# rueberger/MJHMC

Measured on AMD Instinct MI355X. Metric: particle-steps/sec (ndims x nparticles x L), higher is better.
Workload: dtype f64 state (ProductOfT: around the f32 matrix-core force)

## Files before the change

mjhmc_amd/csrc/dense_pot64_kernels.hpp:

```cpp
#pragma once
#ifndef __HIPCC_RTC__
#include <hip/hip_runtime.h>
#endif
#include <stdint.h>

#include "dense_pot.hpp"
#include "dense_pot_tile.hpp"

namespace mjhmc {

template <int NB>
struct DVecN;
template <>
struct DVecN<1> {
  using type = double;
};
template <>
struct DVecN<2> {
  using type = __attribute__((ext_vector_type(2))) double;
};
template <>
struct DVecN<4> {
  using type = __attribute__((ext_vector_type(4))) double;
};
// ... 11 lines not shown
template <int NB>
__device__ __forceinline__ int q_off(int q) { return NB * ((q & 3) + 8 * (q >> 2)); }
template <int NB>
__device__ __forceinline__ const double* lane_row(const double* base, int64_t p, int w, int h) {
  return base + (size_t)p * (128 * NB) + 32 * NB * w + 4 * NB * h;
}
template <int NB>
__device__ __forceinline__ double* lane_row(double* base, int64_t p, int w, int h) {
  return base + (size_t)p * (128 * NB) + 32 * NB * w + 4 * NB * h;
}
template <int NB>
__device__ __forceinline__ typename DVecN<NB>::type dv_load(const double* lrow, int q) {
  return *reinterpret_cast<const typename DVecN<NB>::type*>(lrow + q_off<NB>(q));
}
template <int NB>
__device__ __forceinline__ void dv_store(double* lrow, int q, const typename DVecN<NB>::type& v) {
  *reinterpret_cast<typename DVecN<NB>::type*>(lrow + q_off<NB>(q)) = v;
}

constexpr int kPark = 8;
template <int NB>
struct Shared64 {
  Shared<NB> s;
  double red64[4][kP];
  double zn[128 * NB];
  f32x4 park[kPark / 2][256];
};

template <int NB>
struct Work {
  static constexpr int PB = NB == 1 ? 8 : 16;
  static constexpr int PQ = NB * 8 / PB;
  static constexpr unsigned kArea = 16u * PQ * 64u * PB;
  __amdgpu_buffer_rsrc_t rs;
  unsigned voff;
  static constexpr unsigned xb = 0;
  static constexpr unsigned vb = 4 * kArea;
};
template <int NB>
__device__ __forceinline__ Work<NB> work_of(double* scratch, unsigned wg, int w, int lane) {
  Work<NB> k;
  char* base = (char*)scratch + (size_t)wg * (8 * Work<NB>::kArea);
  k.rs = __builtin_amdgcn_make_buffer_rsrc((void*)base, 0, 8 * Work<NB>::kArea, 0x00020000);
  k.voff = (unsigned)w * Work<NB>::kArea + (unsigned)lane * Work<NB>::PB;
  return k;
}
using uvec4 = __attribute__((ext_vector_type(4))) unsigned;
using uvec2 = __attribute__((ext_vector_type(2))) unsigned;
using f64x2 = __attribute__((ext_vector_type(2))) double;
template <int NB>
__device__ __forceinline__ typename DVecN<NB>::type wk_load(const Work<NB>& k, unsigned area, int q) {
  if constexpr (NB == 1) {
    return __builtin_bit_cast(double, __builtin_amdgcn_raw_buffer_load_b64(k.rs, k.voff, area + (unsigned)q * 512u, 0));
  } else if constexpr (NB == 2) {
    return __builtin_bit_cast(f64x2, __builtin_amdgcn_raw_buffer_load_b128(k.rs, k.voff, area + (unsigned)q * 1024u, 0));
  } else {
    const f64x2 lo = __builtin_bit_cast(f64x2, __builtin_amdgcn_raw_buffer_load_b128(k.rs, k.voff, area + (unsigned)q * 2048u, 0));
    const f64x2 hi = __builtin_bit_cast(f64x2, __builtin_amdgcn_raw_buffer_load_b128(k.rs, k.voff, area + (unsigned)q * 2048u + 1024u, 0));
    typename DVecN<4>::type v;
    v[0] = lo[0];
    v[1] = lo[1];
    v[2] = hi[0];
    v[3] = hi[1];
    return v;
  }
}
template <int NB>
__device__ __forceinline__ void wk_store(const Work<NB>& k, unsigned area, int q, const typename DVecN<NB>::type& v) {
  if constexpr (NB == 1) {
    __builtin_amdgcn_raw_buffer_store_b64(__builtin_bit_cast(uvec2, v), k.rs, k.voff, area + (unsigned)q * 512u, 0);
  } else if constexpr (NB == 2) {
    __builtin_amdgcn_raw_buffer_store_b128(__builtin_bit_cast(uvec4, v), k.rs, k.voff, area + (unsigned)q * 1024u, 0);
  } else {
    f64x2 lo, hi;
    lo[0] = v[0];
    lo[1] = v[1];
    hi[0] = v[2];
    hi[1] = v[3];
    __builtin_amdgcn_raw_buffer_store_b128(__builtin_bit_cast(uvec4, lo), k.rs, k.voff, area + (unsigned)q * 2048u, 0);
    __builtin_amdgcn_raw_buffer_store_b128(__builtin_bit_cast(uvec4, hi), k.rs, k.voff, area + (unsigned)q * 2048u + 1024u, 0);
  }
}

template <int NB>
struct PieceOf {
  using type = uvec4;
};
template <>
struct PieceOf<1> {
  using type = unsigned long long;
};
template <int NB>
struct Stage {
  using P = typename PieceOf<NB>::type;
  static constexpr int PB = sizeof(P);
  static constexpr int RB = 1024 * NB;
  static constexpr int RP = RB / PB;
  static constexpr int K = 32 * RP / 256;
  static constexpr int KB = K < 16 ? K : 16;
};
__device__ __forceinline__ unsigned stage_addr(int row, int piece, int pb, int rb) {
  return (unsigned)(row * rb + ((piece ^ (row & 15)) * pb));
}
template <int NB>
__device__ __forceinline__ void stage_rows_in(const double* rows, int64_t p, char* img) {
  using S = Stage<NB>;
  using P = typename S::P;
  const int t = threadIdx.x;
#pragma unroll 1
  for (int i0 = 0; i0 < S::K; i0 += S::KB) {
    P buf[S::KB];
#pragma unroll
    for (int i = 0; i < S::KB; ++i) {
      const int k = (i0 + i) * 256 + t, row = k / S::RP, piece = k % S::RP;
      const int64_t pr = __shfl((long long)p, row);
      buf[i] = *reinterpret_cast<const P*>(reinterpret_cast<const char*>(rows) + (size_t)pr * S::RB + (size_t)piece * S::PB);
    }
#pragma unroll
    for (int i = 0; i < S::KB; ++i) {
      const int k = (i0 + i) * 256 + t, row = k / S::RP, piece = k % S::RP;
      *reinterpret_cast<P*>(img + stage_addr(row, piece, S::PB, S::RB)) = buf[i];
    }
  }
}
template <int NB>
__device__ __forceinline__ void stage_rows_out(double* rows, int64_t p, const char* img) {
  using S = Stage<NB>;
  using P = typename S::P;
  const int t = threadIdx.x;
#pragma unroll 1
  for (int i0 = 0; i0 < S::K; i0 += S::KB) {
#pragma unroll
    for (int i = 0; i < S::KB; ++i) {
      const int k = (i0 + i) * 256 + t, row = k / S::RP, piece = k % S::RP;
      const int64_t pr = __shfl((long long)p, row);
      *reinterpret_cast<P*>(reinterpret_cast<char*>(rows) + (size_t)pr * S::RB + (size_t)piece * S::PB) =
          *reinterpret_cast<const P*>(img + stage_addr(row, piece, S::PB, S::RB));
    }
  }
}
template <int NB>
__device__ __forceinline__ typename DVecN<NB>::type stage_get(const char* img, int w, int c, int h, int q) {
  using S = Stage<NB>;
  const int first = (8 * NB * (32 * w + acc_row(q, h))) / S::PB;
  if constexpr (NB == 4) {
    const f64x2 lo = *reinterpret_cast<const f64x2*>(img + stage_addr(c, first, S::PB, S::RB));
    const f64x2 hi = *reinterpret_cast<const f64x2*>(img + stage_addr(c, first + 1, S::PB, S::RB));
    typename DVecN<4>::type v;
    v[0] = lo[0];
    v[1] = lo[1];
    v[2] = hi[0];
    v[3] = hi[1];
    return v;
  } else {
    return *reinterpret_cast<const typename DVecN<NB>::type*>(img + stage_addr(c, first, S::PB, S::RB));
  }
}
template <int NB>
__device__ __forceinline__ void stage_put(char* img, int w, int c, int h, int q, const typename DVecN<NB>::type& v) {
  using S = Stage<NB>;
  const int first = (8 * NB * (32 * w + acc_row(q, h))) / S::PB;
  if constexpr (NB == 4) {
    f64x2 lo, hi;
    lo[0] = v[0];
    lo[1] = v[1];
    hi[0] = v[2];
    hi[1] = v[3];
    *reinterpret_cast<f64x2*>(img + stage_addr(c, first, S::PB, S::RB)) = lo;
    *reinterpret_cast<f64x2*>(img + stage_addr(c, first + 1, S::PB, S::RB)) = hi;
  } else {
    *reinterpret_cast<typename DVecN<NB>::type*>(img + stage_addr(c, first, S::PB, S::RB)) = v;
  }
}
template <int NB>
__device__ __forceinline__ char* stage_image(Shared<NB>& s) {
  static_assert(sizeof(s.pub) == 32 * Stage<NB>::RB, "the staging image is the two B-operand images");
  return reinterpret_cast<char*>(&s.pub[0][0]);
}

template <int NB>
struct VTile {
  double b[NB][16];
};

template <int NB, int NKICK>
__device__ __forceinline__ void kick_drift_pass(const Work<NB>& wk, const Tile<NB>& g, VTile<NB>& v, double c, double eps,
                                                PubWave<NB>* pub0, int w, int lane) {
  using DV = typename DVecN<NB>::type;
  DV xa[4], xb[4];
  auto load4 = [&](int q4, DV(&x)[4]) {
#pragma unroll
    for (int qq = 0; qq < 4; ++qq) x[qq] = wk_load<NB>(wk, wk.xb, 4 * q4 + qq);
  };
  auto kick4 = [&](int q4) {
#pragma unroll
    for (int qq = 0; qq < 4; ++qq) {
      const int q = 4 * q4 + qq;
#pragma unroll
      for (int r = 0; r < NB; ++r) {
        const double t = c * (double)g.b[r][q];
        double vv = v.b[r][q];
        vv = vv + t;
        if constexpr (NKICK == 2) vv = vv + t;
        v.b[r][q] = vv;
      }
    }
  };
  auto drift4 = [&](int q4, DV(&x)[4]) {
    f32x4 px[NB];
#pragma unroll
    for (int qq = 0; qq < 4; ++qq) {
      const int q = 4 * q4 + qq;
#pragma unroll
      for (int r = 0; r < NB; ++r) {
        const double xx = dget<NB>(x[qq], r) + eps * v.b[r][q];
        dset<NB>(x[qq], r, xx);
        px[r][qq] = (float)xx;
      }
      wk_store<NB>(wk, wk.xb, q, x[qq]);
    }
    if constexpr (NB == 4) {
      unsigned off = ((wk.voff >> 1) & 0xFFFFC000u) | (wk.voff & 0x3FFu);
      asm volatile("" : "+v"(off));
      char* img = reinterpret_cast<char*>(pub0) + off;
#pragma unroll
      for (int r = 0; r < NB; ++r) *reinterpret_cast<f32x4*>(img + (size_t)(r * 4 + q4) * 1024) = px[r];
    } else {
#pragma unroll
      for (int r = 0; r < NB; ++r) pub0[w].v[r][q4][lane] = px[r];
    }
  };
  load4(0, xa);
  load4(1, xb);
  __builtin_amdgcn_sched_barrier(0);
  kick4(0);
  drift4(0, xa);
  __builtin_amdgcn_sched_barrier(0);
  load4(2, xa);
  __builtin_amdgcn_sched_barrier(0);
  kick4(1);
  drift4(1, xb);
  __builtin_amdgcn_sched_barrier(0);
  load4(3, xb);
  __builtin_amdgcn_sched_barrier(0);
  kick4(2);
  drift4(2, xa);
  __builtin_amdgcn_sched_barrier(0);
  kick4(3);
  drift4(3, xb);
}

template <int NB>
__device__ __forceinline__ double closing_kick(const Tile<NB>& g, VTile<NB>& v, double c) {
  double s = 0.0;
#pragma unroll
  for (int q = 0; q < 16; ++q)
#pragma unroll
    for (int r = 0; r < NB; ++r) {
      const double vv = v.b[r][q] + c * (double)g.b[r][q];
      v.b[r][q] = vv;
      s = s + vv * vv;
    }
  return s;
}

template <int NB, class SH>
__device__ __forceinline__ double column_sum(SH& sh, int w, int c, int h, double part) {
  const double both = swap32_sum(part);
  if (h == 0) sh.red64[w][c] = both;
  __syncthreads();
  const double tot = sh.red64[0][c] + sh.red64[1][c] + sh.red64[2][c] + sh.red64[3][c];
  __syncthreads();
  return tot;
}

template <int NB>
__device__ __forceinline__ void staged_start(Shared<NB>& s, const Work<NB>& wk, const double* xin, const double* vin,
                                             const double* gin, int64_t p, int w, int c, int h, Tile<NB>& g, VTile<NB>& v,
                                             bool neg) {
  char* img = stage_image<NB>(s);
  stage_rows_in<NB>(xin, p, img);
  __syncthreads();
#pragma unroll
  for (int q = 0; q < 16; ++q) wk_store<NB>(wk, wk.xb, q, stage_get<NB>(img, w, c, h, q));
  __syncthreads();
  stage_rows_in<NB>(gin, p, img);
  __syncthreads();
#pragma unroll
  for (int q = 0; q < 16; ++q) {
    const typename DVecN<NB>::type gg = stage_get<NB>(img, w, c, h, q);
#pragma unroll
    for (int r = 0; r < NB; ++r) g.b[r][q] = (float)dget<NB>(gg, r);
  }
  __syncthreads();
  stage_rows_in<NB>(vin, p, img);
  __syncthreads();
#pragma unroll
  for (int q = 0; q < 16; ++q) {
    const typename DVecN<NB>::type vv = stage_get<NB>(img, w, c, h, q);
#pragma unroll
    for (int r = 0; r < NB; ++r) v.b[r][q] = neg ? -dget<NB>(vv, r) : dget<NB>(vv, r);
  }
  __syncthreads();
}

template <int NB>
__device__ __forceinline__ void staged_end_x(Shared<NB>& s, const Work<NB>& wk, double* xout, int64_t p, int w, int c, int h) {
  char* img = stage_image<NB>(s);
#pragma unroll
  for (int q = 0; q < 16; ++q) stage_put<NB>(img, w, c, h, q, wk_load<NB>(wk, wk.xb, q));
  __syncthreads();
  stage_rows_out<NB>(xout, p, img);
  __syncthreads();
}
template <int NB>
__device__ __forceinline__ void staged_end_vg(Shared<NB>& s, double* vout, double* gout, int64_t p, int w, int c, int h,
                                              const VTile<NB>& v, const Tile<NB>& g) {
  using DV = typename DVecN<NB>::type;
  char* img = stage_image<NB>(s);
#pragma unroll
  for (int q = 0; q < 16; ++q) {
    DV vv;
#pragma unroll
    for (int r = 0; r < NB; ++r) dset<NB>(vv, r, v.b[r][q]);
    stage_put<NB>(img, w, c, h, q, vv);
  }
  __syncthreads();
  stage_rows_out<NB>(vout, p, img);
  __syncthreads();
#pragma unroll
  for (int q = 0; q < 16; ++q) {
    DV gg;
#pragma unroll
    for (int r = 0; r < NB; ++r) dset<NB>(gg, r, (double)g.b[r][q]);
    stage_put<NB>(img, w, c, h, q, gg);
  }
  __syncthreads();
  stage_rows_out<NB>(gout, p, img);
  __syncthreads();
}

template <int NB, class XP>
__device__ __forceinline__ double pot64_trajectory(const PotModel& mdl, const XP& xp, AReg<NB>& ar, Shared64<NB>& sh, int w, int c, int h,
                                                   int lane, const Work<NB>& wk, Tile<NB>& g, VTile<NB>& v, int L, double eps,
                                                   double chalf, float* ex) {
  PubWave<NB>* pub0 = sh.s.pub[0];
  kick_drift_pass<NB, 1>(wk, g, v, chalf, eps, pub0, w, lane);
  for (int s = 0; s < L; ++s) {
    [[maybe_unused]] const int stamp_slot = s;
    POT_STAMP(0);
    if constexpr (NB == 4) {
#pragma unroll
      for (int k = 0; k < kPark / 2; ++k) {
        f64x2 two;
        two[0] = v.b[NB - 1][15 - 2 * k];
        two[1] = v.b[NB - 1][14 - 2 * k];
        sh.park[k][threadIdx.x] = __builtin_bit_cast(f32x4, two);
      }
    }
    pot_gradient_published<NB>(mdl, xp, ar, sh.s, w, c, h, lane, g, s == L - 1, ex, s);
    if constexpr (NB == 4) {
#pragma unroll
      for (int k = 0; k < kPark / 2; ++k) {
        const f64x2 two = __builtin_bit_cast(f64x2, sh.park[k][threadIdx.x]);
        v.b[NB - 1][15 - 2 * k] = two[0];
        v.b[NB - 1][14 - 2 * k] = two[1];
      }
#pragma unroll
      for (int r = 0; r < NB; ++r)
#pragma unroll
        for (int q = 0; q < 16; ++q) use_here(v.b[r][q]);
    }
    POT_STAMP(6);
    if (s < L - 1) kick_drift_pass<NB, 2>(wk, g, v, chalf, eps, pub0, w, lane);
    POT_STAMP(7);
  }
  const double part = closing_kick<NB>(g, v, chalf);
  return column_sum<NB>(sh, w, c, h, part) / 2.0;
}


template <int NB>
struct Finish64Shared {
  struct {
    int move[kP];
  } s;
  double red64[4][kP];
  double zn[128 * NB];
};

template <int NB, bool REPLAY, int MODE, bool FIX, class SH>
__device__ __forceinline__ void pot64_finish(const Pot64JumpArgs& a, SH& sh, int64_t p, bool alive, size_t roff, int w, int c,
                                             int h, const VTile<NB>& v, const Tile<NB>& g) {
  using DV = typename DVecN<NB>::type;
  const double* xin = a.X_in + roff;
  const double* vin = a.V_in + roff;
  const double* gin = a.G_in + roff;
  double* xo = a.X_out + roff;
  double* vo = a.V_out + roff;
  double* go = a.G_out + roff;
  const int mv = sh.s.move[c];
  const int k = mv & 3;
  bool take, flip, refresh;
  if constexpr (MODE == kModeControl) {
    const bool accept = k & 1, fl = k & 2;
    take = accept;
    flip = accept != fl;
    refresh = (mv & 4) != 0;
  } else {
    take = k == 0;
    flip = (MODE == kModeCT && k == 0) || k == 1;
    refresh = k == 2;
  }
  const bool tile_refreshes = __ballot(refresh) != 0ull;
  if (!FIX || !take) {
#pragma unroll
    for (int q = 0; q < 16; ++q) {
      DV gg;
      if (take) {
        if constexpr (!FIX) {
          DV vv;
#pragma unroll
          for (int r = 0; r < NB; ++r) {
            dset<NB>(vv, r, flip ? -v.b[r][q] : v.b[r][q]);
            dset<NB>(gg, r, (double)g.b[r][q]);
          }
          dv_store<NB>(vo, q, vv);
        }
      } else {
        gg = dv_load<NB>(gin, q);
        dv_store<NB>(xo, q, dv_load<NB>(xin, q));
      }
      dv_store<NB>(go, q, gg);
    }
  }
  double s2 = 0.0;
  if (!take || (REPLAY && refresh)) {
    const double* vsrc = take ? (const double*)vo : vin;
    const bool fl2 = flip && !take;
    const double* nrow = REPLAY ? lane_row<NB>(a.noise, alive ? p : 0, w, h) : nullptr;
#pragma unroll 1
    for (int q = 0; q < 16; ++q) {
      DV vv = dv_load<NB>(vsrc, q);
      if (fl2) vv = -vv;
      if constexpr (REPLAY) {
        if (refresh) {
          const DV z = dv_load<NB>(nrow, q);
#pragma unroll
          for (int r = 0; r < NB; ++r) {
            const double t = dget<NB>(vv, r) * a.r_keep + dget<NB>(z, r) * a.r_mix;
            dset<NB>(vv, r, t);
            s2 = s2 + t * t;
          }
        }
      }
      dv_store<NB>(vo, q, vv);
    }
// ... 80 lines not shown
```

mjhmc_amd/csrc/dense_pot_tile.hpp:

```cpp
#pragma once
#ifndef __HIPCC_RTC__
#include <hip/hip_runtime.h>
#endif
#include <stdint.h>

#include "dense_pot.hpp"
#include "timing_variants.hpp"

namespace mjhmc {

using f32x16 = __attribute__((ext_vector_type(16))) float;
using f32x4 = __attribute__((ext_vector_type(4))) float;

constexpr int kP = 32;

__device__ __forceinline__ int acc_row(int q, int h) { return (q & 3) + 8 * (q >> 2) + 4 * h; }

template <int NB>
struct Tile {
  f32x16 b[NB];
};

template <int NB>
struct VecN;
// ... 36 lines not shown
template <int NB>
__device__ __forceinline__ void tile_store(float* base, int64_t p, int w, int h, const Tile<NB>& t) {
  using V = typename VecN<NB>::type;
  float* row = base + (size_t)p * (128 * NB) + 32 * NB * w;
#pragma unroll
  for (int q = 0; q < 16; ++q) {
    V v;
#pragma unroll
    for (int r = 0; r < NB; ++r) vset<NB>(v, r, t.b[r][q]);
    *reinterpret_cast<V*>(row + NB * acc_row(q, h)) = v;
  }
}

template <int NB>
struct PubWave {
  f32x4 v[NB][4][64];
};

template <int NB>
__device__ __forceinline__ void publish(PubWave<NB>& dst, int lane, const Tile<NB>& t) {
#pragma unroll
  for (int r = 0; r < NB; ++r)
#pragma unroll
    for (int q4 = 0; q4 < 4; ++q4) {
      f32x4 v;
      v[0] = t.b[r][4 * q4 + 0];
      v[1] = t.b[r][4 * q4 + 1];
      v[2] = t.b[r][4 * q4 + 2];
      v[3] = t.b[r][4 * q4 + 3];
      dst.v[r][q4][lane] = v;
    }
}

template <int NB>
__device__ __forceinline__ void a_chunk_load(const float* mlane, int chunk, typename VecN<NB>::type (&dst)[16]) {
  using V = typename VecN<NB>::type;
  constexpr int DIM = 128 * NB;
  const float* base = mlane + (size_t)(32 * NB * (chunk / NB) + (chunk % NB)) * DIM;
#pragma unroll
  for (int q = 0; q < 16; ++q) dst[q] = *reinterpret_cast<const V*>(base + (size_t)(NB * ((q & 3) + 8 * (q >> 2))) * DIM);
}

template <int NB>
__device__ __forceinline__ typename VecN<NB>::type buf_load(__amdgpu_buffer_rsrc_t r, unsigned voff, unsigned soff) {
  using V = typename VecN<NB>::type;
  if constexpr (NB == 4) return __builtin_bit_cast(V, __builtin_amdgcn_raw_buffer_load_b128(r, voff, soff, 0));
  else if constexpr (NB == 2) return __builtin_bit_cast(V, __builtin_amdgcn_raw_buffer_load_b64(r, voff, soff, 0));
  else return __builtin_bit_cast(V, __builtin_amdgcn_raw_buffer_load_b32(r, voff, soff, 0));
}
template <int NB>
__device__ __forceinline__ __amdgpu_buffer_rsrc_t a_rsrc(const float* M) {
  constexpr int DIM = 128 * NB;
  return __builtin_amdgcn_make_buffer_rsrc((void*)M, 0, DIM * DIM * 4, 0x00020000);
}
template <int NB>
__device__ __forceinline__ void a_chunk_load_buf(__amdgpu_buffer_rsrc_t r, unsigned lane_bytes, int chunk,
                                                 typename VecN<NB>::type (&dst)[16]) {
  constexpr int DIM = 128 * NB;
  const unsigned cbase = (unsigned)(32 * NB * (chunk / NB) + (chunk % NB)) * (unsigned)(DIM * 4);
#pragma unroll
  for (int q = 0; q < 16; ++q) dst[q] = buf_load<NB>(r, lane_bytes, cbase + (unsigned)(NB * ((q & 3) + 8 * (q >> 2)) * DIM * 4));
}

template <int NB>
__device__ __forceinline__ void chunk_mfma(const f32x4* bbase, int chunk, int lane, const typename VecN<NB>::type (&a)[16],
                                           f32x4& bnext, Tile<NB>& acc) {
  constexpr int NG = 16 * NB;
#pragma unroll
  for (int q4 = 0; q4 < 4; ++q4) {
    const f32x4 b4 = bnext;
    const int t = 4 * chunk + q4 + 1;
    bnext = bbase[(size_t)(t < NG ? t : NG - 1) * 64 + lane];
    __builtin_amdgcn_sched_barrier(0);
#pragma unroll
    for (int qq = 0; qq < 4; ++qq) {
#pragma unroll
      for (int r = 0; r < NB; ++r)
        acc.b[r] = __builtin_amdgcn_mfma_f32_32x32x2f32(vget<NB>(a[4 * q4 + qq], r), b4[qq], acc.b[r], 0, 0, 0);
    }
    __builtin_amdgcn_sched_barrier(0);
  }
}

template <int NB>
__device__ __forceinline__ void chunk_mfma_ld(const f32x4* bbase, int chunk, int lane, const typename VecN<NB>::type (&a)[16],
                                              f32x4& bnext, Tile<NB>& acc, __amdgpu_buffer_rsrc_t rs, unsigned lane_bytes,
                                              unsigned cbase, typename VecN<NB>::type (&aload)[16]) {
  constexpr int NG = 16 * NB, DIM = 128 * NB;
#pragma unroll
  for (int q4 = 0; q4 < 4; ++q4) {
    const f32x4 b4 = bnext;
    const int t = 4 * chunk + q4 + 1;
    bnext = bbase[(size_t)(t < NG ? t : NG - 1) * 64 + lane];
    __builtin_amdgcn_sched_barrier(0);
#pragma unroll
    for (int qq = 0; qq < 4; ++qq) {
      const int q = 4 * q4 + qq;
#pragma unroll
      for (int r = 0; r < NB; ++r)
        acc.b[r] = __builtin_amdgcn_mfma_f32_32x32x2f32(vget<NB>(a[q], r), b4[qq], acc.b[r], 0, 0, 0);
      aload[q] = buf_load<NB>(rs, lane_bytes, cbase + (unsigned)(NB * ((q & 3) + 8 * (q >> 2)) * DIM * 4));
      __builtin_amdgcn_sched_barrier(0);
    }
    __builtin_amdgcn_sched_barrier(0);
  }
}

template <int NB>
__device__ __forceinline__ void gemm_dim(const float* __restrict__ M, const float* __restrict__ Mnext, const PubWave<NB>* pub,
                                         int w, int c, int h, int lane, typename VecN<NB>::type (&a0)[16], Tile<NB>& acc) {
  constexpr int DIM = 128 * NB, NCH = 4 * NB;
  const size_t lane_off = (size_t)(4 * NB * h) * DIM + 32 * NB * w + NB * c;
  const unsigned lane_bytes = (unsigned)(lane_off * sizeof(float));
  const __amdgpu_buffer_rsrc_t rM = a_rsrc<NB>(M), rN = a_rsrc<NB>(Mnext);
  const f32x4* bbase = &pub[0].v[0][0][0];
  typename VecN<NB>::type a1[16];
  f32x4 bnext = bbase[lane];
#pragma unroll 1
  for (int chunk = 0; chunk < NCH; chunk += 2) {
    const bool more = chunk + 2 < NCH;
    const int c1 = chunk + 1, c2 = more ? chunk + 2 : 0;
    chunk_mfma_ld<NB>(bbase, chunk, lane, a0, bnext, acc, rM, lane_bytes,
                      (unsigned)(32 * NB * (c1 / NB) + (c1 % NB)) * (unsigned)(DIM * 4), a1);
    chunk_mfma_ld<NB>(bbase, chunk + 1, lane, a1, bnext, acc, more ? rM : rN, lane_bytes,
                      (unsigned)(32 * NB * (c2 / NB) + (c2 % NB)) * (unsigned)(DIM * 4), a0);
  }
}

template <int NB>
struct AReg {
  typename VecN<NB>::type a0[16];
};
template <>
struct AReg<1> {
  float w1[4][16];
  float w2[4][16];
};

template <int NB>
__device__ __forceinline__ void areg_load(const PotModel& mdl, int w, int c, int h, AReg<NB>& ar) {
  if constexpr (NB == 1) {
    const float* m1 = mdl.W1 + (size_t)(4 * h) * 128 + 32 * w + c;
    const float* m2 = mdl.W2T + (size_t)(4 * h) * 128 + 32 * w + c;
#pragma unroll
    for (int chunk = 0; chunk < 4; ++chunk) {
      a_chunk_load<1>(m1, chunk, ar.w1[chunk]);
      a_chunk_load<1>(m2, chunk, ar.w2[chunk]);
    }
  } else {
    a_chunk_load<NB>(mdl.W1 + (size_t)(4 * NB * h) * (128 * NB) + 32 * NB * w + NB * c, 0, ar.a0);
  }
}

template <int NB, bool SECOND>
__device__ __forceinline__ void gemm_any(const PotModel& mdl, AReg<NB>& ar, const PubWave<NB>* pub, int w, int c,
                                         int h, int lane, Tile<NB>& acc) {
  if constexpr (NB == 1) {
    const int kdim = mdl.ndims;
#pragma unroll
    for (int chunk = 0; chunk < 4; ++chunk) {
      const float(&a)[16] = SECOND ? ar.w2[chunk] : ar.w1[chunk];
      const f32x4(*blk)[64] = pub[chunk].v[0];
#pragma unroll
      for (int q4 = 0; q4 < 4; ++q4) {
        if (32 * chunk + 8 * q4 < kdim) {
          const f32x4 b4 = blk[q4][lane];
#pragma unroll
          for (int qq = 0; qq < 4; ++qq)
            acc.b[0] = __builtin_amdgcn_mfma_f32_32x32x2f32(a[4 * q4 + qq], b4[qq], acc.b[0], 0, 0, 0);
        }
      }
    }
  } else {
    gemm_dim<NB>(SECOND ? mdl.W2T : mdl.W1, SECOND ? mdl.W1 : mdl.W2T, pub, w, c, h, lane, ar.a0, acc);
  }
}

template <int NB>
__device__ __forceinline__ void rowvec_load(const float* vec, int w, int h, Tile<NB>& t) {
  using V = typename VecN<NB>::type;
  const float* base = vec + 32 * NB * w;
#pragma unroll
  for (int q = 0; q < 16; ++q) {
    const V v = *reinterpret_cast<const V*>(base + NB * acc_row(q, h));
#pragma unroll
    for (int r = 0; r < NB; ++r) t.b[r][q] = vget<NB>(v, r);
  }
}

__device__ __forceinline__ float half_sum(float s) {
  const auto sw = __builtin_amdgcn_permlane32_swap(__float_as_int(s), __float_as_int(s), false, false);
  return __int_as_float(sw[0]) + __int_as_float(sw[1]);
}

template <int NB>
struct Shared {
  PubWave<NB> pub[2][4];
  float red[2][4][kP];
  int move[kP];
  float cb[128 * NB];
  float zn[128 * NB];
};

template <int NB>
struct FinishShared {
  float red[2][4][kP];
  int move[kP];
  float zn[128 * NB];
};

template <int NB, typename F>
__device__ __forceinline__ void column_normals(const RngKey& key, uint32_t pid, int D, F* zn) {
  const int pair = threadIdx.x;
  if (pair < 64 * NB) {
    double z0, z1;
    normal_pair(key, pid, (uint32_t)pair, z0, z1);
    zn[2 * pair] = 2 * pair < D ? (F)z0 : (F)0;
    zn[2 * pair + 1] = 2 * pair + 1 < D ? (F)z1 : (F)0;
  }
}

template <int NB>
__device__ __forceinline__ void stage_bias(const PotModel& mdl, Shared<NB>& sh) {
  for (int i = threadIdx.x; i < 128 * NB; i += 256) sh.cb[i] = mdl.cb[i];
}


struct PotExperts {
  static constexpr bool kProductOfT = true;
};

template <int NB, class XP>
__device__ __forceinline__ void pot_gradient_published(const PotModel& mdl, const XP& xp, AReg<NB>& ar, Shared<NB>& sh, int w, int c, int h,
                                                       int lane, Tile<NB>& g, bool want_energy, float* energy_out,
                                                       int stamp_slot = 0) {
  __syncthreads();
  POT_STAMP(1);
  Tile<NB> u;
  rowvec_load<NB>(sh.cb, w, h, u);
  gemm_any<NB, false>(mdl, ar, sh.pub[0], w, c, h, lane, u);
  POT_STAMP(2);
  if constexpr (XP::kProductOfT) {
    if (want_energy) {
      using V = typename VecN<NB>::type;
      const float* al = mdl.alpha + 32 * NB * w;
      float s = 0.f;
#pragma unroll
      for (int q = 0; q < 16; ++q) {
        const V a4 = *reinterpret_cast<const V*>(al + NB * acc_row(q, h));
#pragma unroll
        for (int r = 0; r < NB; ++r) s += vget<NB>(a4, r) * logf(1.0f + u.b[r][q] * u.b[r][q]);
      }
      const float part = half_sum(s);
      if (h == 0) sh.red[0][w][c] = part;
    }
#pragma unroll
    for (int r = 0; r < NB; ++r)
#pragma unroll
      for (int q = 0; q < 16; ++q) {
        const float uu = u.b[r][q];
        u.b[r][q] = uu * __builtin_amdgcn_rcpf(1.0f + uu * uu);
      }
  } else {
    if (want_energy) {
      const float part = half_sum(xp.template energy_sum<NB>(u, w, h));
      if (h == 0) sh.red[0][w][c] = part;
    }
    xp.template phi<NB>(u, w, h);
  }
  publish<NB>(sh.pub[1][w], lane, u);
  POT_STAMP(3);
  __syncthreads();
  POT_STAMP(4);
#pragma unroll
  for (int r = 0; r < NB; ++r)
#pragma unroll
    for (int q = 0; q < 16; ++q) g.b[r][q] = 0.f;
  gemm_any<NB, true>(mdl, ar, sh.pub[1], w, c, h, lane, g);
  POT_STAMP(5);
  if (want_energy && energy_out) {
    *energy_out = sh.red[0][0][c] + sh.red[0][1][c] + sh.red[0][2][c] + sh.red[0][3][c];
  }
}

template <int NB, class XP>
__device__ __forceinline__ void pot_gradient(const PotModel& mdl, const XP& xp, AReg<NB>& ar, Shared<NB>& sh, int w, int c, int h,
                                             int lane, const Tile<NB>& x, Tile<NB>& g, bool want_energy,
                                             float* energy_out) {
  [[maybe_unused]] const int stamp_slot = 0;
  POT_STAMP(0);
  publish<NB>(sh.pub[0][w], lane, x);
  pot_gradient_published<NB>(mdl, xp, ar, sh, w, c, h, lane, g, want_energy, energy_out);
}

template <int NB, class SH>
__device__ __forceinline__ float pot_kinetic(SH& sh, int w, int c, int h, const Tile<NB>& v) {
  float s = 0.f;
#pragma unroll
  for (int r = 0; r < NB; ++r)
#pragma unroll
    for (int q = 0; q < 16; ++q) s += v.b[r][q] * v.b[r][q];
  const float part = half_sum(s);
  if (h == 0) sh.red[1][w][c] = part;
  __syncthreads();
  const float tot = (sh.red[1][0][c] + sh.red[1][1][c] + sh.red[1][2][c] + sh.red[1][3][c]) / 2.0f;
  __syncthreads();
  return tot;
}

template <int NB, class XP>
__device__ __forceinline__ void pot_trajectory(const PotModel& mdl, const XP& xp, AReg<NB>& ar, Shared<NB>& sh, int w, int c, int h,
                                               int lane, Tile<NB>& x, Tile<NB>& v, Tile<NB>& g, int L, float eps,
                                               float chalf, float* ex) {
  if (L > 0) {
#pragma unroll
    for (int r = 0; r < NB; ++r)
#pragma unroll
      for (int q = 0; q < 16; ++q) v.b[r][q] = v.b[r][q] + chalf * g.b[r][q];
  }
  for (int s = 0; s < L; ++s) {
#pragma unroll
    for (int r = 0; r < NB; ++r)
#pragma unroll
      for (int q = 0; q < 16; ++q) x.b[r][q] = x.b[r][q] + eps * v.b[r][q];
    pot_gradient<NB>(mdl, xp, ar, sh, w, c, h, lane, x, g, s == L - 1, ex);
    const float ck = s == L - 1 ? chalf : 2.0f * chalf;
#pragma unroll
    for (int r = 0; r < NB; ++r)
#pragma unroll
      for (int q = 0; q < 16; ++q) v.b[r][q] = v.b[r][q] + ck * g.b[r][q];
  }
}

template <int NB>
__device__ __forceinline__ void pot_normals(const RngKey& key, uint32_t pid, int w, int h, int D, Tile<NB>& z) {
#pragma unroll 1
  for (int q = 0; q < 16; ++q) {
    const int d = 32 * NB * w + NB * acc_row(q, h);
    double zz[4] = {0, 0, 0, 0};
    normal_pair(key, pid, (uint32_t)(d >> 1), zz[0], zz[1]);
    if constexpr (NB == 4) normal_pair(key, pid, (uint32_t)((d >> 1) + 1), zz[2], zz[3]);
    if constexpr (NB == 1) {
      z.b[0][q] = d < D ? (float)((d & 1) ? zz[1] : zz[0]) : 0.f;
    } else {
#pragma unroll
      for (int r = 0; r < NB; ++r) z.b[r][q] = d + r < D ? (float)zz[r] : 0.f;
    }
  }
}

}
```

mjhmc_amd/csrc/timing_variants.hpp:

```cpp
#pragma once

#ifdef POT_STAMPS
namespace mjhmc {
static __device__ unsigned long long g_pot_stamp[4][8][8];
}
#define POT_STAMP(I)                                                                                          \
  do {                                                                                                        \
    if (blockIdx.x == 0 && lane == 0) g_pot_stamp[w][stamp_slot & 7][I] = __builtin_readcyclecounter();      \
  } while (0)
namespace mjhmc {
static __device__ unsigned long long g_pot_istamp[4][16][16];
}
#define POT_ISTAMP(I)                                                                                         \
  do {                                                                                                        \
    if (blockIdx.x == 0 && lane == 0 && a.first_pid == 0) {                                                   \
      g_pot_istamp[w][istamp_item][I] = __builtin_readcyclecounter();                                              \
      g_pot_istamp[w][istamp_item][8 + (I)] = __builtin_amdgcn_s_memrealtime();                            \
    }                                                                                                         \
  } while (0)
#else
#define POT_STAMP(I) do { } while (0)
#define POT_ISTAMP(I) do { } while (0)
#endif

#ifdef SIC_STAMPS
namespace mjhmc {
static __device__ unsigned g_sic_stamp[4][8][8];
}
#define SIC_STAMP(RD, I)                                                                                          \
  do {                                                                                                            \
    if (((I) == (SIC_STAMPS) || ((I) == 0 && (RD) == 0)) && blockIdx.x == 0 && lane == 0 && (w & 2) == 0)         \
      sh.stamp[(w & 1) | ((w >> 2) << 1)][RD][I] = (unsigned)__builtin_readcyclecounter();                        \
  } while (0)
#else
#define SIC_STAMP(RD, I) do { } while (0)
#endif

#ifdef ROWS_STAMPS
namespace mjhmc {
static __device__ unsigned long long g_rows_stamp[4][64][16];
}
#define ROWS_STAMP(I)                                                                                                    \
  do {                                                                                                                   \
    if (blockIdx.x == 0 && stamp_on && (threadIdx.x & 63) == 0) g_rows_stamp[threadIdx.x >> 6][stamp_it & 63][I] = __builtin_readcyclecounter(); \
  } while (0)
#else
#define ROWS_STAMP(I) do { } while (0)
#endif
```

mjhmc_amd/csrc/dense_pot64_jump.inc:

```
  __shared__ Shared64<NB> sh;
  if (a.ctl->failed) return;
  const int lane = threadIdx.x & 63, w = threadIdx.x >> 6, c = lane & 31, h = lane >> 5;
  const int ncold = MODE == kModeMJHMC ? *a.cold_count : 0;
  const int64_t nft = (ncold + kP - 1) / kP;
  if ((int64_t)blockIdx.x >= nft + a.ntiles) return;
  if (MODE == kModeMJHMC && blockIdx.x == 0 && threadIdx.x == 0) {
    *a.zero_count = 0;
    if (ncold) atomicAdd(&a.stats[3], (unsigned long long)ncold << 32);
  }
  __shared__ unsigned tally[5];
  if (threadIdx.x < 5) tally[threadIdx.x] = 0;
  AReg<NB> ar;
  areg_load<NB>(mdl, w, c, h, ar);
  stage_bias<NB>(mdl, sh.s);
  const Work<NB> wk = work_of<NB>(a.scratch, blockIdx.x, w, lane);
  for (int64_t item = blockIdx.x; item < nft + a.ntiles; item += gridDim.x) {
    const bool inverse = item < nft;
    [[maybe_unused]] const int istamp_item = (int)(item / gridDim.x) & 15;
    auto column_of = [&](int64_t it) -> int64_t {
      if (it < nft) {
        const int64_t slot = it * kP + c;
        return a.cold_list[slot < ncold ? slot : ncold - 1];
      }
      return (it - nft) * kP + c;
    };
    Tile<NB> g;
    VTile<NB> v;
    float exl = 0.f;
    double EVL;
    {
      const int64_t p = column_of(item);
      POT_ISTAMP(0);
      staged_start<NB>(sh.s, wk, a.X_in, a.V_in, a.G_in, p, w, c, h, g, v, inverse);
      POT_ISTAMP(1);
      EVL = pot64_trajectory<NB>(mdl, xp, ar, sh, w, c, h, lane, wk, g, v, a.L, a.eps, a.chalf, &exl);
      POT_ISTAMP(2);
    }
    int64_t item_again = item;
    asm volatile("" : "+s"(item_again));
    const int64_t p = column_of(item_again);
    const bool alive = p < a.N;
    const size_t roff = (size_t)p * (128 * NB) + 32 * NB * w + 4 * NB * h;
    if (!inverse) staged_end_x<NB>(sh.s, wk, a.X_out, p, w, c, h);
    POT_ISTAMP(3);
    const double EXL = (double)exl;
    const double HL = EXL + EVL;
    if (inverse) {
      if (w == 0 && h == 0) a.Hwork[p] = HL;
      __syncthreads();
      POT_ISTAMP(4);
      continue;
    }

    if constexpr (MODE == kModeMJHMC) {
      if (w == 0 && h == 0) {
        a.EX_out[p] = EXL;
        a.EV_out[p] = EVL;
      }
      staged_end_vg<NB>(sh.s, a.V_out, a.G_out, p, w, c, h, v, g);
      POT_ISTAMP(4);
      continue;
    }

    if (w == 0 && h == 0) {
      const int64_t pp = alive ? p : 0;
      const uint32_t pid = (uint32_t)(a.first_pid + pp);
      const double EX0 = a.EX_in[p], EV0 = a.EV_in[p];
      const double H0 = EX0 + EV0;
      double best = 0.0;
      bool bad = false, gate = false;
      const int k = pot64_decide<REPLAY, MODE>(a, H0, HL, 0.0, pp, pid, best, bad, gate);
      if (bad && alive) tally[4] = 1;
      a.dwell[p] = best;
      a.dwell_ring[p] = best;
      a.trans[p] = (uint8_t)k;
      sh.s.move[c] = k | (gate ? 4 : 0);
      {
        unsigned long long b0, b1, b2, b3 = 0ull;
        if constexpr (MODE == kModeControl) {
          b0 = __ballot(alive && k == 3);
          b1 = __ballot(alive && k == 2);
          b2 = __ballot(alive && gate);
          b3 = __ballot(alive && k == 1);
        } else {
          b0 = __ballot(alive && k == 0);
          b1 = __ballot(alive && k == 1);
          b2 = __ballot(alive && k == 2);
        }
        if (c == 0) {
          if (b0) atomicAdd(&tally[0], (unsigned)__popcll(b0));
          if (b1) atomicAdd(&tally[1], (unsigned)__popcll(b1));
          if (b2) atomicAdd(&tally[2], (unsigned)__popcll(b2));
          if (b3) atomicAdd(&tally[3], (unsigned)__popcll(b3));
        }
      }
      const bool took_L = MODE == kModeControl ? (k & 1) : (k == 0);
      a.EX_out[p] = took_L ? EXL : EX0;
      a.EV_out[p] = took_L ? EVL : EV0;
      a.Hflf_out[p] = __builtin_nan("");
    }
    __syncthreads();
    pot64_finish<NB, REPLAY, MODE, false>(a, sh, p, alive, roff, w, c, h, v, g);
    __syncthreads();
    POT_ISTAMP(4);
  }
  __syncthreads();
  if (threadIdx.x == 0 && tally[4]) {
    a.ctl->failed = 1;
    a.ctl->failed_iter = a.iter;
  }
  if (threadIdx.x < 4 && tally[threadIdx.x]) atomicAdd(&a.stats[threadIdx.x], (unsigned long long)tally[threadIdx.x]);
```

Baseline: 62.27 billion.

## Prefetch f64 position rows into LDS during the last GEMM chunk

For the 512-dimension ProductOfT instance, the second GEMM's final chunk now issues buffer_load...lds requests. These pull the first half of the f64 position tile straight into the wave's publish LDS area. The following kick/drift pass then reads those rows from LDS instead of issuing global loads, hiding their latency behind the MFMA work. The cost is inline-asm exec/m0 manipulation and a hand-tuned vmcnt wait, which couples correctness to the exact number of outstanding loads. It also depends on the publish buffer not being overwritten before the pass consumes it.

Measured after the change: 62.16 billion. No clear change (-0.2%).

```diff
diff --git a/mjhmc_amd/csrc/dense_pot64_kernels.hpp b/mjhmc_amd/csrc/dense_pot64_kernels.hpp
--- a/mjhmc_amd/csrc/dense_pot64_kernels.hpp
+++ b/mjhmc_amd/csrc/dense_pot64_kernels.hpp
@@ -117,6 +117,30 @@
   }
 }
 
+struct XPrefetch {
+  static constexpr bool kActive = true;
+  __amdgpu_buffer_rsrc_t rs;
+  unsigned voff;
+  unsigned lds;
+  bool on;
+  __device__ __forceinline__ void request(int i, unsigned go) const {
+    const unsigned slot = 4u * ((unsigned)(i >> 1) & 3u) + 2u * (unsigned)(i >> 3) + (unsigned)(i & 1);
+    unsigned so;
+    unsigned long long ex;
+    asm volatile(
+        "s_mov_b64 %1, exec\n\ts_cmp_lg_u32 %8, 0\n\ts_cselect_b64 exec, %1, 0\n\t"
+        "s_add_u32 m0, %4, %5\n\ts_movk_i32 %0, %6\n\tbuffer_load_dwordx4 %2, %3, %0 offen lds\n\t"
+        "s_mov_b64 exec, %1"
+        : "=&s"(so), "=&s"(ex)
+        : "v"(voff), "s"(rs), "s"(lds), "i"(slot * 1024u), "i"((unsigned)i * 1024u), "i"(0), "s"(go)
+        : "memory", "m0", "scc");
+  }
+};
+template <int N>
+__device__ __forceinline__ void wait_vmcnt() {
+  asm volatile("s_waitcnt vmcnt(%0)" ::"i"(N) : "memory");
+}
+
 template <int NB>
 struct PieceOf {
   using type = uvec4;
@@ -218,9 +242,10 @@
   double b[NB][16];
 };
 
-template <int NB, int NKICK>
+template <int NB, int NKICK, bool PRE = false>
 __device__ __forceinline__ void kick_drift_pass(const Work<NB>& wk, const Tile<NB>& g, VTile<NB>& v, double c, double eps,
-                                                PubWave<NB>* pub0, int w, int lane) {
+                                                PubWave<NB>* pub0, int w, int lane, [[maybe_unused]] int stamp_slot = 0) {
+  static_assert(!PRE || (NB == 4 && NKICK == 2), "the prefetched pass follows a GEMM 2 of the 512-dimension instance");
   using DV = typename DVecN<NB>::type;
   DV xa[4], xb[4];
   auto load4 = [&](int q4, DV(&x)[4]) {
@@ -265,6 +290,43 @@
       for (int r = 0; r < NB; ++r) pub0[w].v[r][q4][lane] = px[r];
     }
   };
+  if constexpr (PRE) {
+    auto lds4 = [&](int q4, DV(&x)[4]) {
+      unsigned off = ((wk.voff >> 1) & 0xFFFFC000u) | (wk.voff & 0x3FFu);
+      asm volatile("" : "+v"(off));
+      const char* img = reinterpret_cast<const char*>(pub0) + off;
+#pragma unroll
+      for (int qq = 0; qq < 4; ++qq) {
+        const f64x2 lo = *reinterpret_cast<const f64x2*>(img + (size_t)(4 * qq + 2 * q4) * 1024);
+        const f64x2 hi = *reinterpret_cast<const f64x2*>(img + (size_t)(4 * qq + 2 * q4 + 1) * 1024);
+        x[qq][0] = lo[0];
+        x[qq][1] = lo[1];
+        x[qq][2] = hi[0];
+        x[qq][3] = hi[1];
+      }
+    };
+    load4(2, xa);
+    __builtin_amdgcn_sched_barrier(0);
+    wait_vmcnt<8>();
+    __builtin_amdgcn_sched_barrier(0);
+    lds4(0, xb);
+    kick4(0);
+    drift4(0, xb);
+    __builtin_amdgcn_sched_barrier(0);
+    lds4(1, xb);
+    kick4(1);
+    drift4(1, xb);
+    __builtin_amdgcn_sched_barrier(0);
+    load4(3, xb);
+    __builtin_amdgcn_sched_barrier(0);
+    POT_STAMP(8);
+    kick4(2);
+    drift4(2, xa);
+    __builtin_amdgcn_sched_barrier(0);
+    kick4(3);
+    drift4(3, xb);
+    return;
+  }
   load4(0, xa);
   load4(1, xb);
   __builtin_amdgcn_sched_barrier(0);
@@ -380,6 +442,7 @@
                                                    int lane, const Work<NB>& wk, Tile<NB>& g, VTile<NB>& v, int L, double eps,
                                                    double chalf, float* ex) {
   PubWave<NB>* pub0 = sh.s.pub[0];
+  constexpr bool kPre = NB == 4 && XP::kProductOfT;
   kick_drift_pass<NB, 1>(wk, g, v, chalf, eps, pub0, w, lane);
   for (int s = 0; s < L; ++s) {
     [[maybe_unused]] const int stamp_slot = s;
@@ -393,7 +456,17 @@
         sh.park[k][threadIdx.x] = __builtin_bit_cast(f32x4, two);
       }
     }
-    pot_gradient_published<NB>(mdl, xp, ar, sh.s, w, c, h, lane, g, s == L - 1, ex, s);
+    if constexpr (kPre) {
+      XPrefetch pf;
+      pf.rs = wk.rs;
+      pf.voff = wk.voff;
+      pf.lds = __builtin_amdgcn_readfirstlane(
+          (unsigned)(unsigned long)(__attribute__((address_space(3))) const void*)&pub0[w]);
+      pf.on = s < L - 1;
+      pot_gradient_published<NB>(mdl, xp, ar, sh.s, w, c, h, lane, g, s == L - 1, ex, s, pf);
+    } else {
+      pot_gradient_published<NB>(mdl, xp, ar, sh.s, w, c, h, lane, g, s == L - 1, ex, s);
+    }
     if constexpr (NB == 4) {
 #pragma unroll
       for (int k = 0; k < kPark / 2; ++k) {
@@ -407,7 +480,7 @@
         for (int q = 0; q < 16; ++q) use_here(v.b[r][q]);
     }
     POT_STAMP(6);
-    if (s < L - 1) kick_drift_pass<NB, 2>(wk, g, v, chalf, eps, pub0, w, lane);
+    if (s < L - 1) kick_drift_pass<NB, 2, kPre>(wk, g, v, chalf, eps, pub0, w, lane, stamp_slot);
     POT_STAMP(7);
   }
   const double part = closing_kick<NB>(g, v, chalf);
diff --git a/mjhmc_amd/csrc/dense_pot_tile.hpp b/mjhmc_amd/csrc/dense_pot_tile.hpp
--- a/mjhmc_amd/csrc/dense_pot_tile.hpp
+++ b/mjhmc_amd/csrc/dense_pot_tile.hpp
@@ -142,10 +142,15 @@
   }
 }
 
-template <int NB>
+struct NoPrefetch {
+  static constexpr bool kActive = false;
+};
+
+template <int NB, class PF = NoPrefetch, int HALF = 0>
 __device__ __forceinline__ void chunk_mfma_ld(const f32x4* bbase, int chunk, int lane, const typename VecN<NB>::type (&a)[16],
                                               f32x4& bnext, Tile<NB>& acc, __amdgpu_buffer_rsrc_t rs, unsigned lane_bytes,
-                                              unsigned cbase, typename VecN<NB>::type (&aload)[16]) {
+                                              unsigned cbase, typename VecN<NB>::type (&aload)[16], const PF& pf = PF(),
+                                              [[maybe_unused]] unsigned go = 0) {
   constexpr int NG = 16 * NB, DIM = 128 * NB;
 #pragma unroll
   for (int q4 = 0; q4 < 4; ++q4) {
@@ -160,15 +165,19 @@
       for (int r = 0; r < NB; ++r)
         acc.b[r] = __builtin_amdgcn_mfma_f32_32x32x2f32(vget<NB>(a[q], r), b4[qq], acc.b[r], 0, 0, 0);
       aload[q] = buf_load<NB>(rs, lane_bytes, cbase + (unsigned)(NB * ((q & 3) + 8 * (q >> 2)) * DIM * 4));
+      if constexpr (PF::kActive) {
+        if (q & 1) pf.request(8 * HALF + (q >> 1), go);
+      }
       __builtin_amdgcn_sched_barrier(0);
     }
     __builtin_amdgcn_sched_barrier(0);
   }
 }
 
-template <int NB>
+template <int NB, class PF = NoPrefetch>
 __device__ __forceinline__ void gemm_dim(const float* __restrict__ M, const float* __restrict__ Mnext, const PubWave<NB>* pub,
-                                         int w, int c, int h, int lane, typename VecN<NB>::type (&a0)[16], Tile<NB>& acc) {
+                                         int w, int c, int h, int lane, typename VecN<NB>::type (&a0)[16], Tile<NB>& acc,
+                                         const PF& pf = PF()) {
   constexpr int DIM = 128 * NB, NCH = 4 * NB;
   const size_t lane_off = (size_t)(4 * NB * h) * DIM + 32 * NB * w + NB * c;
   const unsigned lane_bytes = (unsigned)(lane_off * sizeof(float));
@@ -180,10 +189,12 @@
   for (int chunk = 0; chunk < NCH; chunk += 2) {
     const bool more = chunk + 2 < NCH;
     const int c1 = chunk + 1, c2 = more ? chunk + 2 : 0;
-    chunk_mfma_ld<NB>(bbase, chunk, lane, a0, bnext, acc, rM, lane_bytes,
-                      (unsigned)(32 * NB * (c1 / NB) + (c1 % NB)) * (unsigned)(DIM * 4), a1);
-    chunk_mfma_ld<NB>(bbase, chunk + 1, lane, a1, bnext, acc, more ? rM : rN, lane_bytes,
-                      (unsigned)(32 * NB * (c2 / NB) + (c2 % NB)) * (unsigned)(DIM * 4), a0);
+    unsigned go = 0;
+    if constexpr (PF::kActive) go = __builtin_amdgcn_readfirstlane(pf.on && !more ? 1u : 0u);
+    chunk_mfma_ld<NB, PF, 0>(bbase, chunk, lane, a0, bnext, acc, rM, lane_bytes,
+                             (unsigned)(32 * NB * (c1 / NB) + (c1 % NB)) * (unsigned)(DIM * 4), a1, pf, go);
+    chunk_mfma_ld<NB, PF, 1>(bbase, chunk + 1, lane, a1, bnext, acc, more ? rM : rN, lane_bytes,
+                             (unsigned)(32 * NB * (c2 / NB) + (c2 % NB)) * (unsigned)(DIM * 4), a0, pf, go);
   }
 }
 
@@ -212,9 +223,9 @@
   }
 }
 
-template <int NB, bool SECOND>
+template <int NB, bool SECOND, class PF = NoPrefetch>
 __device__ __forceinline__ void gemm_any(const PotModel& mdl, AReg<NB>& ar, const PubWave<NB>* pub, int w, int c,
-                                         int h, int lane, Tile<NB>& acc) {
+                                         int h, int lane, Tile<NB>& acc, const PF& pf = PF()) {
   if constexpr (NB == 1) {
     const int kdim = mdl.ndims;
 #pragma unroll
@@ -232,7 +243,7 @@
       }
     }
   } else {
-    gemm_dim<NB>(SECOND ? mdl.W2T : mdl.W1, SECOND ? mdl.W1 : mdl.W2T, pub, w, c, h, lane, ar.a0, acc);
+    gemm_dim<NB, PF>(SECOND ? mdl.W2T : mdl.W1, SECOND ? mdl.W1 : mdl.W2T, pub, w, c, h, lane, ar.a0, acc, pf);
   }
 }
 
@@ -290,10 +301,10 @@
   static constexpr bool kProductOfT = true;
 };
 
-template <int NB, class XP>
+template <int NB, class XP, class PF = NoPrefetch>
 __device__ __forceinline__ void pot_gradient_published(const PotModel& mdl, const XP& xp, AReg<NB>& ar, Shared<NB>& sh, int w, int c, int h,
                                                        int lane, Tile<NB>& g, bool want_energy, float* energy_out,
-                                                       int stamp_slot = 0) {
+                                                       int stamp_slot = 0, const PF& pf = PF()) {
   __syncthreads();
   POT_STAMP(1);
   Tile<NB> u;
@@ -336,7 +347,7 @@
   for (int r = 0; r < NB; ++r)
 #pragma unroll
     for (int q = 0; q < 16; ++q) g.b[r][q] = 0.f;
-  gemm_any<NB, true>(mdl, ar, sh.pub[1], w, c, h, lane, g);
+  gemm_any<NB, true, PF>(mdl, ar, sh.pub[1], w, c, h, lane, g, pf);
   POT_STAMP(5);
   if (want_energy && energy_out) {
     *energy_out = sh.red[0][0][c] + sh.red[0][1][c] + sh.red[0][2][c] + sh.red[0][3][c];
diff --git a/mjhmc_amd/csrc/timing_variants.hpp b/mjhmc_amd/csrc/timing_variants.hpp
--- a/mjhmc_amd/csrc/timing_variants.hpp
+++ b/mjhmc_amd/csrc/timing_variants.hpp
@@ -2,7 +2,7 @@
 
 #ifdef POT_STAMPS
 namespace mjhmc {
-static __device__ unsigned long long g_pot_stamp[4][8][8];
+static __device__ unsigned long long g_pot_stamp[4][8][16];
 }
 #define POT_STAMP(I)                                                                                          \
   do {                                                                                                        \
```

## Software-pipeline staged row loads/stores via buffer ops and merge X write into VG end

Applied to the files above, without the earlier changes.

Row staging in and out of shared memory now uses raw buffer loads and stores with a per-wave row base taken by readlane, in place of per-lane shuffles and flat addressing. On the start path, each next array's global loads are issued while the previous array is being written into the shared image. In MJHMC mode the X output write moves into a combined V/G/X end routine, so the workspace X loads are issued before the G store. Register use goes up because whole rows are held in registers, which may lower occupancy, and the timing stamp macros are generalised along the way.

Result: no change. 62.40 billion before, 62.69 billion after, median of 6 (+0.5%).

```diff
diff --git a/mjhmc_amd/csrc/dense_pot64_jump.inc b/mjhmc_amd/csrc/dense_pot64_jump.inc
--- a/mjhmc_amd/csrc/dense_pot64_jump.inc
+++ b/mjhmc_amd/csrc/dense_pot64_jump.inc
@@ -16,7 +16,7 @@
   const Work<NB> wk = work_of<NB>(a.scratch, blockIdx.x, w, lane);
   for (int64_t item = blockIdx.x; item < nft + a.ntiles; item += gridDim.x) {
     const bool inverse = item < nft;
-    [[maybe_unused]] const int istamp_item = (int)(item / gridDim.x) & 15;
+    [[maybe_unused]] const int istamp_item = blockIdx.x == 0 && a.first_pid == 0 ? (int)(item / gridDim.x) & 15 : -1;
     auto column_of = [&](int64_t it) -> int64_t {
       if (it < nft) {
         const int64_t slot = it * kP + c;
@@ -31,7 +31,7 @@
     {
       const int64_t p = column_of(item);
       POT_ISTAMP(0);
-      staged_start<NB>(sh.s, wk, a.X_in, a.V_in, a.G_in, p, w, c, h, g, v, inverse);
+      staged_start<NB>(sh.s, wk, a.X_in, a.V_in, a.G_in, p, w, c, h, g, v, inverse, istamp_item);
       POT_ISTAMP(1);
       EVL = pot64_trajectory<NB>(mdl, xp, ar, sh, w, c, h, lane, wk, g, v, a.L, a.eps, a.chalf, &exl);
       POT_ISTAMP(2);
@@ -41,8 +41,10 @@
     const int64_t p = column_of(item_again);
     const bool alive = p < a.N;
     const size_t roff = (size_t)p * (128 * NB) + 32 * NB * w + 4 * NB * h;
-    if (!inverse) staged_end_x<NB>(sh.s, wk, a.X_out, p, w, c, h);
-    POT_ISTAMP(3);
+    if (MODE != kModeMJHMC && !inverse) {
+      staged_end_x<NB>(sh.s, wk, a.X_out, p, w, c, h);
+      POT_ISTAMP(3);
+    }
     const double EXL = (double)exl;
     const double HL = EXL + EVL;
     if (inverse) {
@@ -57,7 +59,7 @@
         a.EX_out[p] = EXL;
         a.EV_out[p] = EVL;
       }
-      staged_end_vg<NB>(sh.s, a.V_out, a.G_out, p, w, c, h, v, g);
+      staged_end_vgx<NB>(sh.s, wk, a.V_out, a.G_out, a.X_out, p, w, c, h, v, g, istamp_item);
       POT_ISTAMP(4);
       continue;
     }
diff --git a/mjhmc_amd/csrc/dense_pot64_kernels.hpp b/mjhmc_amd/csrc/dense_pot64_kernels.hpp
--- a/mjhmc_amd/csrc/dense_pot64_kernels.hpp
+++ b/mjhmc_amd/csrc/dense_pot64_kernels.hpp
@@ -138,40 +138,86 @@
   return (unsigned)(row * rb + ((piece ^ (row & 15)) * pb));
 }
 template <int NB>
-__device__ __forceinline__ void stage_rows_in(const double* rows, int64_t p, char* img) {
+struct RowRegs {
+  typename Stage<NB>::P b[Stage<NB>::K];
+};
+__device__ __forceinline__ int stage_thread() {
+  int t = threadIdx.x;
+  asm volatile("" : "+v"(t));
+  return t;
+}
+__device__ __forceinline__ int stage_column(int c) {
+  asm volatile("" : "+v"(c));
+  return c;
+}
+template <int NB>
+__device__ __forceinline__ __amdgpu_buffer_rsrc_t stage_row(const double* rows, int64_t p, int i, int w) {
+  using S = Stage<NB>;
+  const int row = __builtin_amdgcn_readfirstlane((i * 256 + 64 * w) / S::RP);
+  const unsigned lo = (unsigned)__builtin_amdgcn_readlane((int)(unsigned)p, row);
+  const unsigned hi = (unsigned)__builtin_amdgcn_readlane((int)(unsigned)((unsigned long long)p >> 32), row);
+  const size_t pr = ((size_t)hi << 32) | lo;
+  return __builtin_amdgcn_make_buffer_rsrc(const_cast<char*>(reinterpret_cast<const char*>(rows)) + pr * S::RB, 0, S::RB, 0x00020000);
+}
+template <int NB>
+__device__ __forceinline__ typename Stage<NB>::P stage_row_load(__amdgpu_buffer_rsrc_t rs, unsigned off) {
+  if constexpr (NB == 1) return __builtin_bit_cast(unsigned long long, __builtin_amdgcn_raw_buffer_load_b64(rs, off, 0, 0));
+  else return __builtin_bit_cast(uvec4, __builtin_amdgcn_raw_buffer_load_b128(rs, off, 0, 0));
+}
+template <int NB>
+__device__ __forceinline__ void stage_row_store(__amdgpu_buffer_rsrc_t rs, unsigned off, const typename Stage<NB>::P& v) {
+  if constexpr (NB == 1) __builtin_amdgcn_raw_buffer_store_b64(__builtin_bit_cast(uvec2, v), rs, off, 0, 0);
+  else __builtin_amdgcn_raw_buffer_store_b128(v, rs, off, 0, 0);
+}
+template <int NB>
+__device__ __forceinline__ void rows_request(const double* rows, int64_t p, int w, RowRegs<NB>& r) {
+  using S = Stage<NB>;
+  const unsigned off = (unsigned)(stage_thread() % S::RP) * S::PB;
+#pragma unroll
+  for (int i = 0; i < S::K; ++i) r.b[i] = stage_row_load<NB>(stage_row<NB>(rows, p, i, w), off);
+}
+template <int NB>
+__device__ __forceinline__ void rows_to_image(const RowRegs<NB>& r, char* img) {
   using S = Stage<NB>;
   using P = typename S::P;
-  const int t = threadIdx.x;
-#pragma unroll 1
-  for (int i0 = 0; i0 < S::K; i0 += S::KB) {
-    P buf[S::KB];
-#pragma unroll
-    for (int i = 0; i < S::KB; ++i) {
-      const int k = (i0 + i) * 256 + t, row = k / S::RP, piece = k % S::RP;
-      const int64_t pr = __shfl((long long)p, row);
-      buf[i] = *reinterpret_cast<const P*>(reinterpret_cast<const char*>(rows) + (size_t)pr * S::RB + (size_t)piece * S::PB);
-    }
-#pragma unroll
-    for (int i = 0; i < S::KB; ++i) {
-      const int k = (i0 + i) * 256 + t, row = k / S::RP, piece = k % S::RP;
-      *reinterpret_cast<P*>(img + stage_addr(row, piece, S::PB, S::RB)) = buf[i];
-    }
-  }
-}
-template <int NB>
-__device__ __forceinline__ void stage_rows_out(double* rows, int64_t p, const char* img) {
+  const int t = stage_thread();
+#pragma unroll
+  for (int i = 0; i < S::K; ++i) {
+    const int k = i * 256 + t, row = k / S::RP, piece = k % S::RP;
+    *reinterpret_cast<P*>(img + stage_addr(row, piece, S::PB, S::RB)) = r.b[i];
+  }
+}
+template <int NB>
+__device__ __forceinline__ void rows_to_image_request(RowRegs<NB>& r, char* img, const double* next, int64_t p, int w) {
   using S = Stage<NB>;
   using P = typename S::P;
-  const int t = threadIdx.x;
-#pragma unroll 1
-  for (int i0 = 0; i0 < S::K; i0 += S::KB) {
-#pragma unroll
-    for (int i = 0; i < S::KB; ++i) {
+  const int t = stage_thread();
+  const unsigned off = (unsigned)(t % S::RP) * S::PB;
+#pragma unroll
+  for (int i = 0; i < S::K; ++i) {
+    const int k = i * 256 + t, row = k / S::RP, piece = k % S::RP;
+    *reinterpret_cast<P*>(img + stage_addr(row, piece, S::PB, S::RB)) = r.b[i];
+    r.b[i] = stage_row_load<NB>(stage_row<NB>(next, p, i, w), off);
+  }
+}
+template <int NB, int B = Stage<NB>::K>
+__device__ __forceinline__ void stage_rows_out(double* rows, int64_t p, int w, const char* img) {
+  using S = Stage<NB>;
+  using P = typename S::P;
+  static_assert(S::K % B == 0, "whole batches");
+  const int t = stage_thread();
+  const unsigned off = (unsigned)(t % S::RP) * S::PB;
+#pragma unroll
+  for (int i0 = 0; i0 < S::K; i0 += B) {
+    P buf[B];
+#pragma unroll
+    for (int i = 0; i < B; ++i) {
       const int k = (i0 + i) * 256 + t, row = k / S::RP, piece = k % S::RP;
-      const int64_t pr = __shfl((long long)p, row);
-      *reinterpret_cast<P*>(reinterpret_cast<char*>(rows) + (size_t)pr * S::RB + (size_t)piece * S::PB) =
-          *reinterpret_cast<const P*>(img + stage_addr(row, piece, S::PB, S::RB));
-    }
+      buf[i] = *reinterpret_cast<const P*>(img + stage_addr(row, piece, S::PB, S::RB));
+    }
+#pragma unroll
+    for (int i = 0; i < B; ++i) stage_row_store<NB>(stage_row<NB>(rows, p, i0 + i, w), off, buf[i]);
+    if constexpr (B < S::K) __builtin_amdgcn_sched_barrier(0);
   }
 }
 template <int NB>
@@ -312,14 +358,19 @@
 template <int NB>
 __device__ __forceinline__ void staged_start(Shared<NB>& s, const Work<NB>& wk, const double* xin, const double* vin,
                                              const double* gin, int64_t p, int w, int c, int h, Tile<NB>& g, VTile<NB>& v,
-                                             bool neg) {
+                                             bool neg, [[maybe_unused]] int istamp_item = -1) {
   char* img = stage_image<NB>(s);
-  stage_rows_in<NB>(xin, p, img);
+  c = stage_column(c);
+  RowRegs<NB> r;
+  rows_request<NB>(xin, p, w, r);
+  __builtin_amdgcn_sched_barrier(0);
+  rows_to_image_request<NB>(r, img, gin, p, w);
   __syncthreads();
 #pragma unroll
   for (int q = 0; q < 16; ++q) wk_store<NB>(wk, wk.xb, q, stage_get<NB>(img, w, c, h, q));
   __syncthreads();
-  stage_rows_in<NB>(gin, p, img);
+  POT_ISTAMP(5);
+  rows_to_image_request<NB>(r, img, vin, p, w);
   __syncthreads();
 #pragma unroll
   for (int q = 0; q < 16; ++q) {
@@ -328,7 +379,8 @@
     for (int r = 0; r < NB; ++r) g.b[r][q] = (float)dget<NB>(gg, r);
   }
   __syncthreads();
-  stage_rows_in<NB>(vin, p, img);
+  POT_ISTAMP(6);
+  rows_to_image<NB>(r, img);
   __syncthreads();
 #pragma unroll
   for (int q = 0; q < 16; ++q) {
@@ -340,19 +392,54 @@
 }
 
 template <int NB>
+struct XEnd {
+  typename DVecN<NB>::type x[16];
+};
+template <int NB>
+__device__ __forceinline__ void end_x_request(const Work<NB>& wk, XEnd<NB>& xe) {
+#pragma unroll
+  for (int q = 0; q < 16; ++q) xe.x[q] = wk_load<NB>(wk, wk.xb, q);
+  __builtin_amdgcn_sched_barrier(0);
+}
+
+template <int NB>
 __device__ __forceinline__ void staged_end_x(Shared<NB>& s, const Work<NB>& wk, double* xout, int64_t p, int w, int c, int h) {
   char* img = stage_image<NB>(s);
-#pragma unroll
-  for (int q = 0; q < 16; ++q) stage_put<NB>(img, w, c, h, q, wk_load<NB>(wk, wk.xb, q));
-  __syncthreads();
-  stage_rows_out<NB>(xout, p, img);
-  __syncthreads();
-}
-template <int NB>
-__device__ __forceinline__ void staged_end_vg(Shared<NB>& s, double* vout, double* gout, int64_t p, int w, int c, int h,
-                                              const VTile<NB>& v, const Tile<NB>& g) {
+  c = stage_column(c);
+  using DV = typename DVecN<NB>::type;
+  DV xa[4], xb[4];
+  auto load4 = [&](int q4, DV(&x)[4]) {
+#pragma unroll
+    for (int qq = 0; qq < 4; ++qq) x[qq] = wk_load<NB>(wk, wk.xb, 4 * q4 + qq);
+  };
+  auto put4 = [&](int q4, const DV(&x)[4]) {
+#pragma unroll
+    for (int qq = 0; qq < 4; ++qq) stage_put<NB>(img, w, c, h, 4 * q4 + qq, x[qq]);
+  };
+  load4(0, xa);
+  load4(1, xb);
+  __builtin_amdgcn_sched_barrier(0);
+  put4(0, xa);
+  __builtin_amdgcn_sched_barrier(0);
+  load4(2, xa);
+  __builtin_amdgcn_sched_barrier(0);
+  put4(1, xb);
+  __builtin_amdgcn_sched_barrier(0);
+  load4(3, xb);
+  __builtin_amdgcn_sched_barrier(0);
+  put4(2, xa);
+  put4(3, xb);
+  __syncthreads();
+  stage_rows_out<NB, 8>(xout, p, w, img);
+  __syncthreads();
+}
+template <int NB>
+__device__ __forceinline__ void staged_end_vgx(Shared<NB>& s, const Work<NB>& wk, double* vout, double* gout, double* xout,
+                                               int64_t p, int w, int c, int h, const VTile<NB>& v, const Tile<NB>& g,
+                                               [[maybe_unused]] int istamp_item = -1) {
   using DV = typename DVecN<NB>::type;
   char* img = stage_image<NB>(s);
+  c = stage_column(c);
 #pragma unroll
   for (int q = 0; q < 16; ++q) {
     DV vv;
@@ -361,8 +448,9 @@
     stage_put<NB>(img, w, c, h, q, vv);
   }
   __syncthreads();
-  stage_rows_out<NB>(vout, p, img);
-  __syncthreads();
+  stage_rows_out<NB>(vout, p, w, img);
+  __syncthreads();
+  POT_ISTAMP(7);
 #pragma unroll
   for (int q = 0; q < 16; ++q) {
     DV gg;
@@ -370,8 +458,17 @@
     for (int r = 0; r < NB; ++r) dset<NB>(gg, r, (double)g.b[r][q]);
     stage_put<NB>(img, w, c, h, q, gg);
   }
-  __syncthreads();
-  stage_rows_out<NB>(gout, p, img);
+  __builtin_amdgcn_sched_barrier(0);
+  XEnd<NB> xe;
+  end_x_request<NB>(wk, xe);
+  __syncthreads();
+  stage_rows_out<NB>(gout, p, w, img);
+  __syncthreads();
+  POT_ISTAMP(3);
+#pragma unroll
+  for (int q = 0; q < 16; ++q) stage_put<NB>(img, w, c, h, q, xe.x[q]);
+  __syncthreads();
+  stage_rows_out<NB>(xout, p, w, img);
   __syncthreads();
 }
 
diff --git a/mjhmc_amd/csrc/timing_variants.hpp b/mjhmc_amd/csrc/timing_variants.hpp
--- a/mjhmc_amd/csrc/timing_variants.hpp
+++ b/mjhmc_amd/csrc/timing_variants.hpp
@@ -13,9 +13,9 @@
 }
 #define POT_ISTAMP(I)                                                                                         \
   do {                                                                                                        \
-    if (blockIdx.x == 0 && lane == 0 && a.first_pid == 0) {                                                   \
-      g_pot_istamp[w][istamp_item][I] = __builtin_readcyclecounter();                                              \
-      g_pot_istamp[w][istamp_item][8 + (I)] = __builtin_amdgcn_s_memrealtime();                            \
+    if (istamp_item >= 0 && (threadIdx.x & 63) == 0) {                                                        \
+      g_pot_istamp[threadIdx.x >> 6][istamp_item][I] = __builtin_readcyclecounter();                          \
+      g_pot_istamp[threadIdx.x >> 6][istamp_item][8 + (I)] = __builtin_amdgcn_s_memrealtime();                \
     }                                                                                                         \
   } while (0)
 #else
```
